# imazen/imageflow

Hardware: NVIDIA B200
Metric: input Mpixels/s, c2_4k_to_512_robidoux (higher is better)
Workload: dtype f32

## Files before the change

imageflow_b200/csrc/ifb_engine.cu:

```cuda
#include <cuda_runtime.h>

#include <algorithm>
#include <atomic>
#include <chrono>
#include <condition_variable>
#include <thread>
#include <cmath>
#include <cstdarg>
#include <cstdio>
#include <cstring>
#include <map>
#include <memory>
#include <mutex>
#include <set>
#include <stdexcept>
#include <string>
#include <tuple>
#include <unordered_map>
#include <vector>

#include "../../include/ifb200.h"
#include "ifb_kernels.cuh"
#include "ifb_weights.h"
#include "ifb_whitespace.h"
// ... 85 lines not shown
    size_t add(const void* src, size_t bytes) {
        const size_t off = (host.size() + 255) / 256 * 256;
        host.resize(off + bytes);
        if (bytes && src) memcpy(host.data() + off, src, bytes);
        return off;
    }
    template <class T> size_t add(const std::vector<T>& v) { return add(v.data(), v.size() * sizeof(T)); }
    size_t add_zeroed(size_t bytes) { return add(nullptr, bytes); }
    template <class T> T* host_at(size_t off) { return reinterpret_cast<T*>(host.data() + off); }
    void reserve(size_t bytes) { host.reserve(bytes); }
    void commit(ifb200_batch* b, cudaStream_t st);
    void use_on(cudaStream_t st) {
        if (done || st == up_stream) return;
        if (cudaEventQuery(ready) == cudaSuccess) { done = true; return; }
        CUDA_OK(cudaStreamWaitEvent(st, ready, 0));
    }
    template <class T> const T* at(size_t off) const { return reinterpret_cast<const T*>(p + off); }
    ~DevBlob() { if (ready && owns_ready) cudaEventDestroy(ready); }
    DevBlob() = default;
    DevBlob(const DevBlob&) = delete;
    DevBlob& operator=(const DevBlob&) = delete;
};

struct AxisOnDev {
    size_t o_left = 0, o_right = 0, o_off = 0, o_w = 0;
    void add_to(DevBlob& blob, const ifb::AxisWeights& a) { o_left = blob.add(a.left); o_right = blob.add(a.right); o_off = blob.add(a.offset); o_w = blob.add(a.w); }
    AxisDev view(const DevBlob& blob) const { return AxisDev{blob.at<uint32_t>(o_left), blob.at<uint32_t>(o_right), blob.at<uint32_t>(o_off), blob.at<float>(o_w)}; }
};

struct HvTables {
    int max_cols = 0, n_strips = 0;
    uint32_t hw_stride = 0;
    std::vector<HvStripDev> strips;
    DevBlob blob;
    size_t o_strips = 0, o_hw = 0, o_hdone = 0, o_vw = 0, o_vdone = 0;
};

struct Plan {
    uint32_t in_w, in_h, out_w, out_h;
    ifb::AxisWeights wv, wh;
    AxisOnDev dv, dh; std::unique_ptr<DevBlob> axes;
    bool tile_ok = false; TilePlanDev tile{};
    std::vector<float> tile_vw, tile_hw; std::vector<uint32_t> tile_vq; size_t o_tile_vw = 0, o_tile_vq = 0, o_tile_hw = 0;
    bool hv_ok = false; std::string hv_reason;
    int av = 0;
    std::map<int, std::unique_ptr<HvTables>> by_cols;
    std::vector<int> cols_failed;
};

bool monotone(const ifb::AxisWeights& a) {
    for (uint32_t i = 1; i < a.out_size; ++i)
        if (a.left[i] < a.left[i - 1] || a.right[i] < a.right[i - 1]) return false;
    return true;
}

int ring_depth(const ifb::AxisWeights& a) {
    int need = 1;
    for (; need <= 64; ++need) {
        bool ok = true;
        for (uint32_t y = 0; y + need < a.out_size && ok; ++y) ok = a.left[y + need] > a.right[y];
        if (ok) break;
    }
    return need;
}

void build_hv(Plan& p) {
// ... 15 lines not shown
        t.max_ic = std::max<int>(t.max_ic, (int)(p.wh.right[X1 - 1] - p.wh.left[X0] + 1));
    }
    for (int ty = 0; ty < t.tiles_y; ++ty) {
        const uint32_t Y0 = ty * t.toh, Y1 = std::min<uint32_t>(Y0 + t.toh, p.out_h);
        t.max_ir = std::max<int>(t.max_ir, (int)(p.wv.right[Y1 - 1] - p.wv.left[Y0] + 1));
    }
    if (Tile2Smem::make(t.max_ir, t.max_ic, true).total > 96u * 1024u) return;
    const int rows_pad = t.tiles_y * kTile2H;
    p.tile_vw.assign((size_t)rows_pad * 8, 0.0f);
    p.tile_vq.assign((size_t)rows_pad / 4, 0u);
    for (int ty = 0; ty < t.tiles_y; ++ty) {
        const uint32_t Y0 = ty * t.toh, Y1 = std::min<uint32_t>(Y0 + t.toh, p.out_h);
        const uint32_t r0 = p.wv.left[Y0], r1 = p.wv.right[Y1 - 1];
        for (uint32_t yq = Y0; yq < Y1; yq += 4) {
            const uint32_t b0 = std::min(p.wv.left[yq], std::max(r1 - std::min<uint32_t>(r1, kTile2Span - 1), r0));
            bool fit = r1 - r0 + 1 >= (uint32_t)kTile2Span;
            for (uint32_t y = yq; y < std::min(yq + 4, Y1); ++y) fit = fit && p.wv.left[y] >= b0 && p.wv.right[y] < b0 + kTile2Span;
            p.tile_vq[yq / 4] = fit ? b0 + 1 : 0u;
            if (!fit) continue;
            for (uint32_t y = yq; y < std::min(yq + 4, Y1); ++y)
                for (uint32_t j = p.wv.left[y]; j <= p.wv.right[y]; ++j) p.tile_vw[(size_t)y * 8 + (j - b0)] = p.wv.w[p.wv.offset[y] + (j - p.wv.left[y])];
        }
    }
    t.h4 = p.wh.max_taps <= 4 ? 1 : 0;
    p.tile_hw.assign(t.h4 ? (size_t)t.tiles_x * kTile2W * 4 : 4, 0.0f);
    if (t.h4)
        for (uint32_t x = 0; x < p.out_w; ++x)
            for (uint32_t j = p.wh.left[x]; j <= p.wh.right[x]; ++j) p.tile_hw[(size_t)x * 4 + (j - p.wh.left[x])] = p.wh.w[p.wh.offset[x] + (j - p.wh.left[x])];
    p.tile = t; p.tile_ok = true;
}

template <class F> void hv_for_av(int av, F&& f) { if (av == 4) f(std::integral_constant<int, 4>{}); else f(std::integral_constant<int, 6>{}); }

std::unique_ptr<HvTables> hv_tables_host(const Plan& p, int cols_key) {
    auto ht = std::make_unique<HvTables>();
    const int max_cols = cols_key & 0xffff, ng = cols_key >> 16, cg = 32 / (p.av / 2);
    ht->max_cols = max_cols;
    const auto& h = p.wh; const auto& v = p.wv;
    const int av = p.av, avp = av == 4 ? 4 : 8, cap = 16384 / (avp * 4);
    const uint32_t col_cap = (uint32_t)max_cols;
    static const uint32_t k0_align = [] { const char* e = getenv("IFB200_DEBUG_K0_ALIGN"); const int v = e ? atoi(e) : 4; return (uint32_t)(v >= 1 && v <= 16 ? v : 4); }();
    auto k0_of = [&](uint32_t X0) { return h.left[X0] / k0_align * k0_align; };
    auto marks_of = [&](uint32_t X0, uint32_t X1, std::vector<uint32_t>* marks) {
        const uint32_t k0 = k0_of(X0);
        uint32_t parked = 0, X = X0, groups = 0;
        const uint32_t npairs = (h.right[X1 - 1] - k0 + 1 + 15) / 16 * 2;
        for (uint32_t c = 0; c < npairs; ++c) {
            uint32_t m = 0;
            while (X < X1 && h.right[X] <= k0 + c * 8 + 7) { ++m; ++X; }
            if (m > (uint32_t)cg) return false;
            if (parked + m > (uint32_t)cg) { if (marks) marks->push_back(c - 1); ++groups; parked = 0; }
            parked += m;
        }
        if (parked) { if (marks) marks->push_back(npairs - 1); ++groups; }
        return groups <= (uint32_t)ng;
    };
    auto fits = [&](uint32_t X0, uint32_t X1) {
        return X1 - X0 <= col_cap && (h.right[X1 - 1] - k0_of(X0) + 1 + 15) / 16 * 16 + 16 <= (uint32_t)cap && marks_of(X0, X1, nullptr);
    };
    uint32_t ns = 0;
    for (uint32_t X0 = 0; X0 < h.out_size; ++ns) {
        uint32_t X1 = X0 + 1;
        if (!fits(X0, X1)) IFB_THROW(IFB200_ERR_INVALID_STATE, "ring kernel: one output column reads %u source columns (> %d)", h.right[X0] - h.left[X0] + 1, cap - 16);
        while (X1 < h.out_size && fits(X0, X1 + 1)) ++X1;
        X0 = X1;
    }
    std::vector<HvStripDev>& strips = ht->strips;
    for (;; ++ns) {
        strips.clear();
        bool ok = true;
        for (uint32_t s = 0; s < ns && ok; ++s) {
            const uint32_t X0 = (uint32_t)((uint64_t)h.out_size * s / ns), X1 = (uint32_t)((uint64_t)h.out_size * (s + 1) / ns);
            if (X1 <= X0) { ok = false; break; }
            ok = fits(X0, X1);
            HvStripDev sd{};
            sd.X0 = (int)X0; sd.X1 = (int)X1; sd.k0 = (int)k0_of(X0);
            sd.nst = (int)((h.right[X1 - 1] - k0_of(X0) + 1 + 15) / 16);
            sd.Xf = (int)X0; sd.hslot0 = (int)(X0 % (uint32_t)av);
            strips.push_back(sd);
        }
        if (ok) break;
        if (ns > h.out_size) IFB_THROW(IFB200_ERR_INVALID_STATE, "ring kernel: strip partition failed");
    }
    ht->n_strips = (int)ns;
    uint32_t rec = 0;
    for (const auto& sd : strips) rec = std::max<uint32_t>(rec, (uint32_t)sd.nst * 16u + 16u);
    ht->hw_stride = rec;
    const size_t hd_stride = (size_t)rec + 64;
    ht->blob.reserve(ns * (sizeof(HvStripDev) + (size_t)rec * avp * 4 + hd_stride) + ((size_t)p.in_h + 32) * (avp * 4 + 1) + 4096);
    ht->o_strips = ht->blob.add(strips);
    ht->o_hw = ht->blob.add_zeroed((size_t)ns * rec * avp * sizeof(float));
    ht->o_hdone = ht->blob.add_zeroed((size_t)ns * hd_stride);
    ht->o_vw = ht->blob.add_zeroed(((size_t)p.in_h + 32) * avp * sizeof(float));
    ht->o_vdone = ht->blob.add_zeroed((size_t)p.in_h + 32);
    float* const hw = ht->blob.host_at<float>(ht->o_hw);
    uint8_t* const hdone = ht->blob.host_at<uint8_t>(ht->o_hdone);
    float* const vw = ht->blob.host_at<float>(ht->o_vw);
    uint8_t* const vdone = ht->blob.host_at<uint8_t>(ht->o_vdone);
    std::vector<uint32_t> marks;
    for (uint32_t s = 0; s < ns; ++s) {
        const HvStripDev& sd = strips[s];
        const uint32_t k0 = (uint32_t)sd.k0;
        for (uint32_t X = (uint32_t)sd.X0; X < (uint32_t)sd.X1; ++X) {
            const float* w = h.w.data() + h.offset[X];
            const uint32_t slot = X % (uint32_t)av;
            for (uint32_t k = h.left[X]; k <= h.right[X]; ++k) hw[((size_t)s * rec + (k - k0)) * avp + slot] = w[k - h.left[X]];
            uint8_t& d = hdone[(size_t)s * hd_stride + (h.right[X] - k0)];
            if (d == 127) IFB_THROW(IFB200_ERR_INVALID_STATE, "ring kernel: too many columns complete at once");
            ++d;
        }
        marks.clear();
        marks_of((uint32_t)sd.X0, (uint32_t)sd.X1, &marks);
        for (uint32_t c : marks) hdone[(size_t)s * hd_stride + c * 8 + 7] |= 0x80u;
    }
    for (uint32_t y = 0; y < v.out_size; ++y) {
        const float* w = v.w.data() + v.offset[y];
        const uint32_t slot = y % (uint32_t)av;
        for (uint32_t j = v.left[y]; j <= v.right[y]; ++j) vw[(size_t)j * avp + slot] = w[j - v.left[y]];
        uint8_t& d = vdone[v.right[y]];
        if (d == 255) IFB_THROW(IFB200_ERR_INVALID_STATE, "ring kernel: too many rows complete at once");
        ++d;
    }
    return ht;
}

bool hv_host_ready(Plan& p, int max_cols) {
    if (!p.hv_ok) return false;
    if (p.by_cols.count(max_cols)) return true;
    if (std::find(p.cols_failed.begin(), p.cols_failed.end(), max_cols) != p.cols_failed.end()) return false;
    try { p.by_cols.emplace(max_cols, hv_tables_host(p, max_cols)); return true; }
    catch (const Err& e) { p.cols_failed.push_back(max_cols); if (p.hv_reason.empty()) p.hv_reason = e.msg; return false; }
}

HvTables& hv_tables(ifb200_batch* bt, cudaStream_t st, Plan& p, int max_cols) {
    auto it = p.by_cols.find(max_cols);
    if (it == p.by_cols.end()) it = p.by_cols.emplace(max_cols, hv_tables_host(p, max_cols)).first;
    HvTables& ht = *it->second;
    if (!ht.blob.p) ht.blob.commit(bt, st); else ht.blob.use_on(st);
    return ht;
}

std::vector<HvBandDev> hv_bands(const Plan& p, int nb) {
    const auto& v = p.wv;
    std::vector<HvBandDev> bands;
    for (int i = 0; i < nb; ++i) {
        const uint32_t Y0 = (uint32_t)((uint64_t)p.out_h * i / nb), Y1 = (uint32_t)((uint64_t)p.out_h * (i + 1) / nb);
// ... 416 lines not shown
            if (g.kind == 1) {
                bl = &p.by_cols.at(g.cols_key)->blob;
            } else {
                if (!p.axes) make_axes_blob(p);
                bl = p.axes.get();
            }
            if (!bl->p && !bl->host.empty() && seen.insert(bl).second) cold.push_back(bl);
        }
    }
    size_t cold_next = 0;
    auto upload_ahead = [&](cudaStream_t up) {
        const size_t end = std::min(cold.size(), cold_next + 128);
        if (cold_next < end) { b->commit_many(up, std::vector<DevBlob*>(cold.begin() + cold_next, cold.begin() + end)); cold_next = end; }
    };
    struct GroupLayout { size_t jobs = 0, tmaps = 0, bands = 0, counters = 0; int nb = 0, grid = 0; std::vector<HvBandDev> bv; };
    std::vector<GroupLayout> lay(groups.size());
    size_t bytes = 0;
    auto take = [&](size_t nbytes) { const size_t o = (bytes + 127) / 128 * 128; bytes = o + nbytes; return o; };
    for (size_t gi = 0; gi < groups.size(); ++gi) {
        Group& g = groups[gi];
        lay[gi].jobs = take(g.idx.size() * sizeof(JobDev));
        if (g.kind == 1) {
            Plan& p = *g.plan;
            const HvEntry* he = find_hv(p.av, g.ch);
            const HvTables& ht = *p.by_cols.at(g.cols_key);
            const size_t jxs = g.idx.size() * (size_t)ht.n_strips;
            const int warps_all = b->sm_count * he->warps;
            const int nb = hv_pick_bands(p, jxs, warps_all, b->min_items);
            lay[gi].bv = hv_bands(p, nb);
            lay[gi].nb = (int)lay[gi].bv.size();
            const size_t items = jxs * nb;
            lay[gi].grid = (int)std::min<size_t>((size_t)b->sm_count, (items + he->warps - 1) / he->warps);
            lay[gi].tmaps = take(g.idx.size() * sizeof(HvTmap));
            lay[gi].bands = take(lay[gi].bv.size() * sizeof(HvBandDev));
            lay[gi].counters = take((size_t)ht.n_strips * sizeof(uint32_t));
        }
    }
    cudaEvent_t ev;
    uint8_t* hbuf = static_cast<uint8_t*>(b->stage(bytes, &ev));
    for (size_t gi = 0; gi < groups.size(); ++gi) {
        Group& g = groups[gi];
        JobDev* hj = reinterpret_cast<JobDev*>(hbuf + lay[gi].jobs);
        HvTmap* ht = g.kind == 1 ? reinterpret_cast<HvTmap*>(hbuf + lay[gi].tmaps) : nullptr;
        size_t pos = 0;
        for (size_t i : g.idx) {
            hj[pos] = make_job(descs[i], g_t_lin_host, g_t_srgb_host);
            if (ht) { uint32_t xoff = 0; ht[pos] = tmap_for(b, descs[i], &xoff); hj[pos].in_xoff = xoff; }
            ++pos;
        }
        if (g.kind == 1) {
            memcpy(hbuf + lay[gi].bands, lay[gi].bv.data(), lay[gi].bv.size() * sizeof(HvBandDev));
            memset(hbuf + lay[gi].counters, 0, (size_t)g.plan->by_cols.at(g.cols_key)->n_strips * sizeof(uint32_t));
        }
    }
    uint8_t* dbuf = nullptr;
    CUDA_OK(cudaMallocAsync(reinterpret_cast<void**>(&dbuf), bytes, st));
    AsyncFree dbuf_guard{dbuf, st};
    CUDA_OK(cudaMemcpyAsync(dbuf, hbuf, bytes, cudaMemcpyHostToDevice, st));
    CUDA_OK(cudaEventRecord(ev, st));

    const bool fork = groups.size() >= 4;
    cudaStream_t const user_stream = st;
    if (fork) {
        CUDA_OK(cudaEventRecord(b->ev_fork, user_stream));
        for (auto& sd : b->side) CUDA_OK(cudaStreamWaitEvent(sd, b->ev_fork, 0));
    }
    struct Join {
        ifb200_batch* b; cudaStream_t user; bool on;
        ~Join() {
            if (!on) return;
            for (int k = 0; k < ifb200_batch::kSideStreams; ++k)
                if (cudaEventRecord(b->ev_join[k], b->side[k]) == cudaSuccess) cudaStreamWaitEvent(user, b->ev_join[k], 0);
        }
    } join{b, user_stream, fork};
    for (size_t gi = 0; gi < groups.size(); ++gi) {
        Group& g = groups[gi];
        Plan& p = *g.plan;
        {
            const DevBlob* need = g.kind == 1 ? &p.by_cols.at(g.cols_key)->blob : p.axes.get();
            while (need && !need->p && cold_next < cold.size()) upload_ahead(user_stream);
        }
        const JobDev* jobs = reinterpret_cast<const JobDev*>(dbuf + lay[gi].jobs);
        const size_t nj = g.idx.size();
        st = fork ? b->side[gi % ifb200_batch::kSideStreams] : user_stream;
// ... 465 lines not shown
                    }
                }
            } catch (const Err& e) { errs[me] = e; }
        };
        const auto t0 = std::chrono::steady_clock::now();
        std::vector<std::thread> pool;
        try { for (int t = 1; t < threads; ++t) pool.emplace_back(worker, t); } catch (...) {}
        worker(0);
        for (auto& th : pool) th.join();
        const double dt = std::chrono::duration<double>(std::chrono::steady_clock::now() - t0).count();
        for (auto& e : errs) if (e.code) throw e;
        if (seconds) *seconds = dt;
        if (table_bytes) *table_bytes = bytes.load();
        if (table_hash) { uint64_t h = 14695981039346656037ull; *table_hash = fnv(h, hashes.data(), hashes.size() * 8); }
    });
}

int ifb200_hv_plan_tables(const ifb200_resample_desc* d, int strip_cols, int n_pairs, ifb200_hv_plan_info* info, uint8_t* buf, size_t cap,
                          char* err, size_t err_cap) {
    return guarded(err, err_cap, [&] {
        if (!d || !info) IFB_THROW(IFB200_ERR_INVALID_ARGUMENT, "null pointer");
        if (strip_cols < 16 || strip_cols > 128 || strip_cols % 16 || n_pairs < 1) IFB_THROW(IFB200_ERR_INVALID_ARGUMENT, "bad strip width or band count");
        memset(info, 0, sizeof *info);
        auto p = ifb200_batch::build_plan_host(*d, strip_cols);
        if (!p->hv_ok) return;
        const int cols = hv_cols(p->av, d->alpha_meaningful ? 4 : 3, strip_cols);
        if (!p->by_cols.count(cols)) return;
        HvTables& ht = *p->by_cols.at(cols);
        const std::vector<HvBandDev> bands = hv_bands(*p, n_pairs);
        const size_t o_bands = (ht.blob.host.size() + 255) / 256 * 256;
        info->ok = 1; info->av = p->av; info->n_strips = ht.n_strips; info->n_bands = (int32_t)bands.size();
        info->avp = p->av == 4 ? 4 : 8; info->cap_px = (int32_t)ht.hw_stride;
        info->o_strips = ht.o_strips; info->o_hw = ht.o_hw; info->o_hdone = ht.o_hdone; info->o_vw = ht.o_vw; info->o_vdone = ht.o_vdone;
        info->o_bands = o_bands; info->total = o_bands + bands.size() * sizeof(HvBandDev);
        if (!buf) return;
        if (cap < info->total) IFB_THROW(IFB200_ERR_CAPACITY, "buffer of %zu bytes, %llu needed", cap, (unsigned long long)info->total);
        memcpy(buf, ht.blob.host.data(), ht.blob.host.size());
        memcpy(buf + o_bands, bands.data(), bands.size() * sizeof(HvBandDev));
    });
}

int  ifb200_color_filter_matrix(int which, float p, float out[25]) { return out ? ifb::color_filter_matrix(which, p, out) : IFB200_ERR_INVALID_ARGUMENT; }

int ifb200_batch_create(int device, ifb200_batch** out, char* err, size_t cap) {
    return guarded(err, cap, [&] {
        if (!out) IFB_THROW(IFB200_ERR_INVALID_ARGUMENT, "null out pointer");
        *out = nullptr;
        *out = create_batch(device);
    });
}

int ifb200_batch_enqueue(ifb200_batch* b, const ifb200_resample_desc* descs, size_t n, void* stream, char* err, size_t cap) {
    return guarded(err, cap, [&] {
        if (!b || (!descs && n)) IFB_THROW(IFB200_ERR_INVALID_ARGUMENT, "null batch or descriptor array");
        std::lock_guard<std::mutex> lk(b->mu);
        enqueue_locked(b, descs, n, stream == IFB200_STREAM_OWN ? b->own_stream : static_cast<cudaStream_t>(stream));
    });
}

int ifb200_batch_color_matrix(ifb200_batch* b, uint8_t* dev_px, uint32_t w, uint32_t h, uint32_t stride, const float m[25],
                              void* stream, char* err, size_t cap) {
    return guarded(err, cap, [&] {
        if (!b) IFB_THROW(IFB200_ERR_INVALID_ARGUMENT, "null batch");
        std::lock_guard<std::mutex> lk(b->mu);
        color_matrix_locked(b, dev_px, w, h, stride, m, stream == IFB200_STREAM_OWN ? b->own_stream : static_cast<cudaStream_t>(stream));
    });
}

int ifb200_batch_apply_matte(ifb200_batch* b, uint8_t* dev_px, uint32_t w, uint32_t h, uint32_t stride, const uint8_t matte_bgra[4],
                             int alpha_meaningful, void* stream, char* err, size_t cap) {
    return guarded(err, cap, [&] {
// ... 362 lines not shown
```

imageflow_b200/csrc/ifb_hv_kernel.cuh:

```cuda
#pragma once

#ifndef IFB_HV_EMU
#include <cuda.h>
#endif

struct HvStripDev { int X0, X1, Xf, hslot0, k0, nst, pad0, pad1; };
struct HvBandDev  { int Y0, Y1, Yf, vslot0, j0, nrows, pad0, pad1; };
struct HvPlanDev {
    uint32_t in_w, in_h, out_w, out_h;
    int n_strips, n_bands;
    const HvStripDev* strips;
    const HvBandDev* bands;
    const float* hw;
    const uint8_t* hdone;
    const float* vw;
    const uint8_t* vdone;
    uint32_t zero;
    uint32_t hw_stride;
};
struct alignas(64) HvTmap { unsigned char bytes[128]; };

#ifndef IFB_HV_MAXCOLS4
#define IFB_HV_MAXCOLS4 64
#endif
template <int AV, int CH> struct HvCfg {
    static_assert(AV == 4 || AV == 6, "ring depth");
    static constexpr int kAvp = AV == 4 ? 4 : 8;
    static constexpr int kCapPx = 16384 / (kAvp * 4);
    static constexpr int kNP = AV / 2;
    static constexpr int kCG = 32 / kNP;
    static constexpr int kMaxCols = AV == 4 ? IFB_HV_MAXCOLS4 : (CH == 3 ? 50 : 40);
    static constexpr int kNG = kMaxCols / kCG + 1;
    static constexpr int kWarps = CH == 3 ? 16 : 12;
    static constexpr int kThreads = kWarps * 32;
    static constexpr int kStages = 2;
    static constexpr int kBoxBytes = 32 * 64;
    static constexpr int kStageBytes = kBoxBytes;
    static constexpr int kRingBytes = kStages * kStageBytes;
    static constexpr int kXPitch = CH * 32 + 2;
    static constexpr int kXBytes = kCG * kXPitch * 4;
};

template <int AV, int CH>
__host__ __device__ constexpr uint32_t hv_layout(uint32_t sb_low16, int warp, uint32_t* st_off, uint32_t* x_off, uint32_t* mb_off) {
    using C = HvCfg<AV, CH>;
    const uint32_t lut_off = (0x10000u - sb_low16) & 0xffffu;
    const uint32_t ring = (uint32_t)C::kRingBytes, xb = (uint32_t)C::kXBytes, W = (uint32_t)C::kWarps;
    const uint32_t a0 = (512u - (sb_low16 & 511u)) & 511u;
    const uint32_t roomA = lut_off > a0 ? lut_off - a0 : 0u;
    uint32_t ra = 0, xa = 0, best = 0;
    for (uint32_t r = 0; r <= W; ++r) {
        if (r * ring > roomA) break;
        uint32_t x = (roomA - r * ring) / xb;
        if (x > W) x = W;
        const uint32_t used = r * ring + x * xb;
        if (used > best) { best = used; ra = r; xa = x; }
    }
    const uint32_t b0 = lut_off + 65536u;
    const uint32_t b_x = b0 + (W - ra) * ring;
    const uint32_t b_mb = (b_x + (W - xa) * xb + 7u) & ~7u;
    if (warp >= 0) {
        const uint32_t w = (uint32_t)warp;
        if (st_off) *st_off = w < ra ? a0 + w * ring : b0 + (w - ra) * ring;
        if (x_off) *x_off = w < xa ? a0 + ra * ring + w * xb : b_x + (w - xa) * xb;
        if (mb_off) *mb_off = b_mb + w * 8u * (uint32_t)C::kStages;
    }
    return b_mb + W * 8u * (uint32_t)C::kStages + 16u;
}
template <int AV, int CH> __host__ __device__ constexpr uint32_t hv_flag_offset(uint32_t sb_low16) { return hv_layout<AV, CH>(sb_low16, -1, nullptr, nullptr, nullptr) - 16u; }
template <int AV, int CH> constexpr uint32_t hv_total_bytes(uint32_t sb_low16) { return hv_layout<AV, CH>(sb_low16, -1, nullptr, nullptr, nullptr); }

#ifndef IFB_HV_EMU
namespace hv {
__device__ __forceinline__ uint32_t smem_u32(const void* p) { return (uint32_t)__cvta_generic_to_shared(p); }
// ... 188 lines not shown
    const uint32_t lane4 = ((uint32_t)lane * 4u) | ((lut >> 16) << 8);
    const uint32_t swz = (((uint32_t)lane >> 1) & 3u) << 4;
    const uint32_t n_bands = (uint32_t)pl.n_bands;
    const uint32_t n_items = n_jobs * n_bands;
    const uint32_t lutw = lut + 128u * 256u + 128u;
    const bool leader = hv::elect_one();
    const uint32_t vh = (uint32_t)lane / (uint32_t)CG, cl = (uint32_t)lane % (uint32_t)CG;
    const bool vlane = vh < (uint32_t)NP;
    const uint32_t xr = xbuf + cl * kXCol;
    const uint32_t xw0 = xbuf + (uint32_t)lane * 4u;

    for (int sv = 0; sv < pl.n_strips; ++sv) {
        if (warp == 0) {
            const int k = sv + lane;
            const bool work = k < pl.n_strips && hv::ldg_volatile(counters + (blockIdx.x + (uint32_t)k) % (uint32_t)pl.n_strips) < n_items;
            const uint32_t m = hv::ballot(work);
            if (lane == 0) hv::sts_u32(flagw, m ? (uint32_t)__ffs((int)m) : (sv + 32 < pl.n_strips ? 33u : 0u));
        }
        hv::cta_sync();
        const uint32_t skip1 = hv::lds_u32(flagw);
        hv::cta_sync();
        if (skip1 == 0u) break;
        if (skip1 == 33u) { sv += 31; continue; }
        sv += (int)skip1 - 1;
        const int s = (int)((blockIdx.x + (uint32_t)sv) % (uint32_t)pl.n_strips);
        const HvStripDev sd_ = pl.strips[s];
        const int sX0 = (int)uni((uint32_t)sd_.X0);
        const uint32_t sH0 = uni((uint32_t)sd_.hslot0);
        const int sK0 = (int)uni((uint32_t)sd_.k0), nst = (int)uni((uint32_t)sd_.nst);
        {
            const float4* __restrict__ src = reinterpret_cast<const float4*>(pl.hw + (size_t)s * pl.hw_stride * AVP);
            const int n16 = (nst * 16 + 4) * AVP / 4;
            for (int u = t; u < n16; u += C::kThreads) hv::sts_f32x4(lutw + ((uint32_t)(u >> 3) << 8) + ((uint32_t)(u & 7) << 4), hv::ldg(src + u));
        }
        hv::cta_sync();
        const uint8_t* __restrict__ hdone = pl.hdone + (size_t)s * (pl.hw_stride + 64u);
        const uint32_t npairs = (uint32_t)nst * 2u;

        for (;;) {
            uint32_t item = 0;
            if (lane == 0) item = hv::atomic_inc(counters + s);
            item = uni(hv::bcast0(item));
            if (item >= n_items) break;
            const uint32_t job_i = item / n_bands, band_i = item - job_i * n_bands;
            const JobDev& job = jobs[job_i];
            const HvTmap* tm = tmaps + job_i;
            const HvBandDev bd_ = pl.bands[band_i];
            const int bJ0 = (int)uni((uint32_t)bd_.j0), bNr = (int)uni((uint32_t)bd_.nrows);
            const int bY0 = (int)uni((uint32_t)bd_.Y0), bY1 = (int)uni((uint32_t)bd_.Y1);
            const uint32_t flags = uni(job.flags);
            const int nrb = (bNr + 31) >> 5;
            const int x_origin = sK0 + (int)uni(job.in_xoff);

            const int x_end = x_origin + nst * 16;
            int tma_x = x_origin, tma_y = bJ0, tma_left = nrb * nst, is_s = 0;
            auto issue = [&](const uint32_t zero_dep) {
                hv::warp_sync();
                if (leader) {
                    const uint32_t bar = mb + 8u * (uint32_t)is_s;
                    hv::mbar_expect_tx(bar, (uint32_t)C::kStageBytes);
                    hv::tma_load_box(stb + (uint32_t)is_s * C::kStageBytes, tm, tma_x + (int)zero_dep, tma_y, bar);
                }
                --tma_left; is_s ^= 1;
                tma_x += 16;
                if (tma_x == x_end) { tma_x = x_origin; tma_y += 32; }
            };
// ... 28 lines not shown
                uint32_t wcur = lutw;

                if (tma_left > 0) issue(0u);
                hv::mbar_wait(mb + 8u * (uint32_t)cs_s, (par >> cs_s) & 1u);
                par ^= 1u << cs_s;
                uint32_t sbase = stb + (uint32_t)cs_s * C::kStageBytes + (uint32_t)lane * 64u;
                uint4 rawA = hv::lds_u32x4(sbase + swz), rawB;
                uint32_t hd_next = (uint32_t)hv::ldg(hdone + lane);
                uint32_t HM1 = 0, HM2 = 0, HMV = 0;

                float P0[CH], P1[CH];
                float2 W0[NP], W1[NP];
                auto conv = [&](float (&P)[CH], const uint32_t v) {
                    P[0] = hv::lut_gather<0x6504>(v, lane4); P[1] = hv::lut_gather<0x6514>(v, lane4); P[2] = hv::lut_gather<0x6524>(v, lane4);
                    if (CH == 4) {
                        const float af = __fmul_rn(__uint2float_rn(v >> 24), 1.0f / 255.0f);
                        P[0] = __fmul_rn(P[0], af); P[1] = __fmul_rn(P[1], af); P[2] = __fmul_rn(P[2], af); P[CH - 1] = af;
                    }
                };
                auto wload = [&](float2 (&W)[NP], const uint32_t a) {
                    const float4 q4 = hv::lds_w4(a);
                    W[0] = make_float2(q4.x, q4.y); W[1] = make_float2(q4.z, q4.w);
                    if (AV == 6) W[NP - 1] = hv::lds_w2(a + 16u);
                };
                auto mac = [&](const float (&P)[CH], const float2 (&W)[NP]) {
#pragma unroll
                    for (int c = 0; c < CH; ++c) {
                        const float2 v_ = make_float2(P[c], P[c]);
#pragma unroll
                        for (int q = 0; q < NP; ++q) accH[c][q] = hv::ffma2(W[q], v_, accH[c][q]);
                    }
                };
                wload(W0, wcur); conv(P0, rawA.x);

                for (uint32_t pq = 0; pq < npairs; pq += 4u) {
                    HM1 = hv::ballot((hd_next & 0x7fu) >= 1u); HM2 = hv::ballot((hd_next & 0x7fu) >= 2u); HMV = hv::ballot((hd_next & 0x80u) != 0u);
                    hd_next = (uint32_t)hv::ldg(hdone + (pq + 4u) * 8u + (uint32_t)lane);
                    const uint32_t pe = min(pq + 4u, npairs);
#pragma unroll 1
                  for (uint32_t pc = pq; pc < pe; ++pc) {
                    const uint32_t hm = HM1, hm2 = HM2, hmv = HMV;
                    HM1 >>= 8; HM2 >>= 8; HMV >>= 8;
                    const uint32_t wB = wcur + (AV == 4 ? 64u : 256u);
                    const uint32_t wnext = wcur + (AV == 4 ? 256u : 512u);
                    const bool more = pc + 1u < npairs;

#define IFB_HV_SLOT(S_) case S_: if (S_ < AV) { _Pragma("unroll") for (int ch_ = 0; ch_ < CH; ++ch_) { \
        float& a_ = (S_ & 1) ? accH[ch_][(S_ % AV) / 2].y : accH[ch_][(S_ % AV) / 2].x; \
        hv::sts_f32(xw + (uint32_t)ch_ * 128u, a_); a_ = 0.0f; } } break;
#define IFB_HV_FLUSH(I_) if ((hm >> (I_)) & 1u) { \
        uint32_t n_ = 1u; \
        if ((hm2 >> (I_)) & 1u) n_ = uni((uint32_t)hv::ldg(hdone + pc * 8u + (I_)) & 0x7fu); \
        _Pragma("unroll 1") do { \
            switch (hslot) { IFB_HV_SLOT(0) IFB_HV_SLOT(1) IFB_HV_SLOT(2) IFB_HV_SLOT(3) IFB_HV_SLOT(4) IFB_HV_SLOT(5) default: break; } \
            xw += kXCol; ++colbuf; hslot = hslot + 1u == (uint32_t)AV ? 0u : hslot + 1u; \
        } while (--n_); }

                    rawB = hv::lds_u32x4(sbase + (((((pc & 1u) << 1) | 1u) << 4) ^ swz));
                    if ((pc & 1u) && more) {
                        cs_s ^= 1;
                        if (tma_left > 0) issue(hv::zero_after(rawB.x, pl.zero));
                        hv::mbar_wait(mb + 8u * (uint32_t)cs_s, (par >> cs_s) & 1u);
                        par ^= 1u << cs_s;
                        sbase = stb + (uint32_t)cs_s * C::kStageBytes + (uint32_t)lane * 64u;
                    }
#define IFB_HV_RELOAD rawA = hv::lds_u32x4(sbase + (((((pc + 1u) & 1u) << 1) << 4) ^ swz));
#define IFB_HV_ACC(S_, C_) (((S_) & 1) ? accH[C_][((S_) % AV) / 2].y : accH[C_][((S_) % AV) / 2].x)
#define IFB_HV_PF(S_, BIT_, M_) { \
        if (CH == 3) hv::flush3_if<BIT_, kXCol>(xw, IFB_HV_ACC(S_, 0), IFB_HV_ACC(S_, 1), IFB_HV_ACC(S_, 2), M_); \
        else hv::flush4_if<BIT_, kXCol>(xw, IFB_HV_ACC(S_, 0), IFB_HV_ACC(S_, 1), IFB_HV_ACC(S_, 2), IFB_HV_ACC(S_, CH - 1), M_); }
#define IFB_HV_NONE
#define IFB_HV_STEPS_A(F0_, F1_, F2_, F3_) { \
        wload(W1, wcur + kRec); conv(P1, rawA.y); mac(P0, W0); F0_ \
        wload(W0, wcur + 2u * kRec); conv(P0, rawA.z); mac(P1, W1); F1_ \
        wload(W1, wcur + 3u * kRec); conv(P1, rawA.w); mac(P0, W0); F2_ \
        wload(W0, wB); conv(P0, rawB.x); mac(P1, W1); F3_ }
#define IFB_HV_STEPS_B(F0_, F1_, F2_, F3_) { \
        wload(W1, wB + kRec); conv(P1, rawB.y); mac(P0, W0); F0_ \
        wload(W0, wB + 2u * kRec); conv(P0, rawB.z); mac(P1, W1); F1_ \
        wload(W1, wB + 3u * kRec); conv(P1, rawB.w); IFB_HV_RELOAD mac(P0, W0); F2_ \
        wload(W0, wnext); conv(P0, rawA.x); mac(P1, W1); F3_ }
#define IFB_HV_CHUNK(STEPS_, SH_) { \
        const uint32_t m4_ = (hm >> (SH_)) & 15u; \
        if (IFB_HV_NOFAST || ((((hm2 >> (SH_)) & 15u) | (m4_ & (m4_ - 1u))) != 0u)) { \
            STEPS_(IFB_HV_FLUSH((SH_) + 0), IFB_HV_FLUSH((SH_) + 1), IFB_HV_FLUSH((SH_) + 2), IFB_HV_FLUSH((SH_) + 3)) \
        } else if (m4_ == 0u) { \
            STEPS_(IFB_HV_NONE, IFB_HV_NONE, IFB_HV_NONE, IFB_HV_NONE) \
        } else { \
            if (hslot < 2u) { \
                if (hslot == 0u) IFB_HV_FORM(STEPS_, 0) else IFB_HV_FORM(STEPS_, 1) \
            } else if (AV == 4 || hslot < 4u) { \
                if (hslot == 2u) IFB_HV_FORM(STEPS_, 2) else IFB_HV_FORM(STEPS_, 3) \
            } else { \
                if (hslot == 4u) IFB_HV_FORM(STEPS_, 4) else IFB_HV_FORM(STEPS_, 5) \
            } \
            ++colbuf; hslot = hslot + 1u == (uint32_t)AV ? 0u : hslot + 1u; \
        } }
#define IFB_HV_FORM(STEPS_, K_) STEPS_(IFB_HV_PF((K_) % AV, 1u, m4_), IFB_HV_PF((K_) % AV, 2u, m4_), IFB_HV_PF((K_) % AV, 4u, m4_), IFB_HV_PF((K_) % AV, 8u, m4_))
                    IFB_HV_CHUNK(IFB_HV_STEPS_A, 0)
                    IFB_HV_CHUNK(IFB_HV_STEPS_B, 4)
#undef IFB_HV_CHUNK
#undef IFB_HV_FORM
#undef IFB_HV_STEPS_A
#undef IFB_HV_STEPS_B
#undef IFB_HV_NONE
#undef IFB_HV_PF
#undef IFB_HV_ACC
#undef IFB_HV_RELOAD
#undef IFB_HV_FLUSH
#undef IFB_HV_SLOT
                    wcur = wnext;

                    if ((hmv >> 7) & 1u) {
                        hv::warp_sync();
                        const bool col_live = vlane && cl < colbuf;
                        uint8_t* const out_px = out_col + (size_t)gX * 4;
                        float2 acc[CH];
                        switch (grp) {
#define IFB_HV_VGROUP(G_) case G_: if (G_ < NG) { _Pragma("unroll") for (int ch_ = 0; ch_ < CH; ++ch_) acc[ch_] = accV[(G_) % NG][ch_]; } break;
                        IFB_HV_VGROUP(0) IFB_HV_VGROUP(1) IFB_HV_VGROUP(2) IFB_HV_VGROUP(3) IFB_HV_VGROUP(4) IFB_HV_VGROUP(5) IFB_HV_VGROUP(6) IFB_HV_VGROUP(7) IFB_HV_VGROUP(8)
#undef IFB_HV_VGROUP
                        default:
#pragma unroll
                            for (int ch_ = 0; ch_ < CH; ++ch_) acc[ch_] = make_float2(0.0f, 0.0f);
                            break;
                        }
                        {
                            int Yb = Yc;
                            uint32_t nc = 0;
                            uint32_t vs = vslot;
                            auto drain = [&]() {
                                hv::warp_sync();
#pragma unroll 1
                                for (uint32_t k0 = 0; k0 < nc; k0 += (uint32_t)NP) {
                                    const uint32_t k = k0 + (vlane ? vh : 0u);
                                    float f_[4] = {0.0f, 0.0f, 0.0f, 0.0f};
#pragma unroll
                                    for (int ch_ = 0; ch_ < CH; ++ch_) f_[ch_] = hv::lds_f32(xr + (uint32_t)ch_ * 128u + (k & 31u) * 4u);
                                    const int Yl = Yb + (int)k;
                                    const bool mine = k < nc && Yl >= bY0 && Yl < bY1 && col_live;
                                    uint8_t* dst = out_px + (size_t)Yl * out_stride;
                                    if (EPI != 0) {
                                        const uint32_t px_ = hv_finish_pixel<EPI, CH>(f_[0], f_[1], f_[2], CH == 4 ? f_[3] : 0.0f, flags, job, lut, lut_lane, dst);
                                        if (mine) *reinterpret_cast<uint32_t*>(dst) = px_;
                                    } else if (mine) {
                                        *reinterpret_cast<uint32_t*>(dst) = hv_finish_pixel<EPI, CH>(f_[0], f_[1], f_[2], CH == 4 ? f_[3] : 0.0f, flags, job, lut, lut_lane, dst);
// ... 31 lines not shown
                                if (n & 1) { vrow(vwp, xrr); vwp += AVP; xrr += 4u; }
                                if (rest != 0u) {
                                    uint32_t nv = 1u;
                                    if (vm2 != 0u && ((vm2 >> (r - 1)) & 1u)) nv = uni((uint32_t)hv::ldg(pl.vdone + row0 + r - 1));
#pragma unroll 1
                                    for (uint32_t e2 = 0; e2 < nv; ++e2) {
                                        if (nc >= (uint32_t)r) drain();
                                        hv::warp_sync();
                                        const bool holder = (vs >> 1) == vh;
                                        const uint32_t pa = xr + nc * 4u;
                                        if (vs & 1u) {
#pragma unroll
                                            for (int ch_ = 0; ch_ < CH; ++ch_) if (holder) { hv::sts_f32(pa + (uint32_t)ch_ * 128u, acc[ch_].y); acc[ch_].y = 0.0f; }
                                        } else {
#pragma unroll
                                            for (int ch_ = 0; ch_ < CH; ++ch_) if (holder) { hv::sts_f32(pa + (uint32_t)ch_ * 128u, acc[ch_].x); acc[ch_].x = 0.0f; }
                                        }
                                        ++nc; vs = vs + 1u == (uint32_t)AV ? 0u : vs + 1u;
                                    }
                                }
                            }
                            drain();
                        }
                        switch (grp) {
#define IFB_HV_VGROUP(G_) case G_: if (G_ < NG) { _Pragma("unroll") for (int ch_ = 0; ch_ < CH; ++ch_) accV[(G_) % NG][ch_] = acc[ch_]; } break;
                        IFB_HV_VGROUP(0) IFB_HV_VGROUP(1) IFB_HV_VGROUP(2) IFB_HV_VGROUP(3) IFB_HV_VGROUP(4) IFB_HV_VGROUP(5) IFB_HV_VGROUP(6) IFB_HV_VGROUP(7) IFB_HV_VGROUP(8)
#undef IFB_HV_VGROUP
                        default: break;
                        }
                        hv::warp_sync();
                        ++grp; gX += colbuf; colbuf = 0; xw = xw0;
                    }
                  }
                }
                cs_s ^= 1;
                Yc += (int)vtot;
                vslot = (vslot + vtot) % (uint32_t)AV;
            }
        }
    }
}
```

Measured before the change: 586,800.

## Add periodic-run fast path with compile-time column completion pattern in HV kernel

On the host, each strip's column-completion pattern is scanned for long runs that match precomputed periodic forms for the 4-tap case. The run offset and length are stored next to the band table. Inside a matched run, the kernel switches to a fully unrolled path whose parking slots are known at compile time, replacing the per-pair ballot masks and runtime branch dispatch. This is meant to cut control overhead in the inner horizontal loop. The cost is larger code and more complex loop bookkeeping, and it only helps when a strip's pattern matches one of the hard-coded forms.

After: 622,100 (median of 6 runs). 1.06x the previous value.

```diff
diff --git a/imageflow_b200/csrc/ifb_engine.cu b/imageflow_b200/csrc/ifb_engine.cu
--- a/imageflow_b200/csrc/ifb_engine.cu
+++ b/imageflow_b200/csrc/ifb_engine.cu
@@ -141,6 +141,7 @@
     int max_cols = 0, n_strips = 0;
     uint32_t hw_stride = 0;
     std::vector<HvStripDev> strips;
+    std::vector<uint32_t> runs;
     DevBlob blob;
     size_t o_strips = 0, o_hw = 0, o_hdone = 0, o_vw = 0, o_vdone = 0;
 };
@@ -222,6 +223,42 @@
 
 template <class F> void hv_for_av(int av, F&& f) { if (av == 4) f(std::integral_constant<int, 4>{}); else f(std::integral_constant<int, 6>{}); }
 
+void hv_find_run(const uint8_t* hd, uint32_t npairs, uint32_t hslot0, int av, int cg, int ng, uint32_t run[2]) {
+    auto pair_done = [&](uint32_t c) { uint32_t d = 0; for (int i = 0; i < 8; ++i) d += hd[c * 8 + i] & 0x7fu; return d; };
+    auto groups_with = [&](uint32_t a, uint32_t P, uint32_t n) {
+        uint32_t parked = 0, groups = 0;
+        for (uint32_t c = 0; c < npairs; ++c) {
+            if (c == a && parked) return -1;
+            parked += pair_done(c);
+            const bool in = c >= a && c < a + n * P;
+            if ((in && (c + 1 - a) % P == 0) || (!in && (hd[c * 8 + 7] & 0x80u) && parked)) { ++groups; parked = 0; }
+        }
+        return (int)groups;
+    };
+    uint32_t best_pairs = 0;
+    for (int f = 0; f < kHvNumForms; ++f) {
+        const HvForm& fm = kHvForms[f];
+        const uint32_t P = (uint32_t)fm.pairs;
+        int tot = 0;
+        for (int i = 0; i < fm.pairs * 8; ++i) tot += fm.cnt[i] - '0';
+        if (fm.av != av || tot > cg) continue;
+        auto period_at = [&](uint32_t c) {
+            for (uint32_t i = 0; i < P * 8; ++i) if ((hd[c * 8 + i] & 0x7fu) != (uint32_t)(fm.cnt[i] - '0')) return false;
+            return true;
+        };
+        uint32_t done = 0;
+        for (uint32_t a = 0; a + P <= npairs; done += pair_done(a), ++a) {
+            if ((hslot0 + done) % (uint32_t)av != (uint32_t)fm.slot) continue;
+            uint32_t n = 0;
+            while (a + (n + 1) * P <= npairs && period_at(a + n * P)) ++n;
+            if (n * P <= best_pairs) continue;
+            const int g = groups_with(a, P, n);
+            if (g < 0 || g > ng) continue;
+            best_pairs = n * P; run[0] = a | (uint32_t)f << 16; run[1] = n;
+        }
+    }
+}
+
 std::unique_ptr<HvTables> hv_tables_host(const Plan& p, int cols_key) {
     auto ht = std::make_unique<HvTables>();
     const int max_cols = cols_key & 0xffff, ng = cols_key >> 16, cg = 32 / (p.av / 2);
@@ -231,6 +268,8 @@
     const uint32_t col_cap = (uint32_t)max_cols;
     static const uint32_t k0_align = [] { const char* e = getenv("IFB200_DEBUG_K0_ALIGN"); const int v = e ? atoi(e) : 4; return (uint32_t)(v >= 1 && v <= 16 ? v : 4); }();
     auto k0_of = [&](uint32_t X0) { return h.left[X0] / k0_align * k0_align; };
+    const char* const pe_ = getenv("IFB200_DEBUG_HV_PERIODIC");
+    const bool periodic = !(pe_ && atoi(pe_) == 0);
     auto marks_of = [&](uint32_t X0, uint32_t X1, std::vector<uint32_t>* marks) {
         const uint32_t k0 = k0_of(X0);
         uint32_t parked = 0, X = X0, groups = 0;
@@ -273,6 +312,7 @@
         if (ns > h.out_size) IFB_THROW(IFB200_ERR_INVALID_STATE, "ring kernel: strip partition failed");
     }
     ht->n_strips = (int)ns;
+    ht->runs.assign(2 * (size_t)ns, 0u);
     uint32_t rec = 0;
     for (const auto& sd : strips) rec = std::max<uint32_t>(rec, (uint32_t)sd.nst * 16u + 16u);
     ht->hw_stride = rec;
@@ -302,6 +342,7 @@
         marks.clear();
         marks_of((uint32_t)sd.X0, (uint32_t)sd.X1, &marks);
         for (uint32_t c : marks) hdone[(size_t)s * hd_stride + c * 8 + 7] |= 0x80u;
+        if (periodic) hv_find_run(hdone + (size_t)s * hd_stride, (uint32_t)sd.nst * 2u, (uint32_t)sd.hslot0, av, cg, ng, &ht->runs[2 * s]);
     }
     for (uint32_t y = 0; y < v.out_size; ++y) {
         const float* w = v.w.data() + v.offset[y];
@@ -784,7 +825,7 @@
             const size_t items = jxs * nb;
             lay[gi].grid = (int)std::min<size_t>((size_t)b->sm_count, (items + he->warps - 1) / he->warps);
             lay[gi].tmaps = take(g.idx.size() * sizeof(HvTmap));
-            lay[gi].bands = take(lay[gi].bv.size() * sizeof(HvBandDev));
+            lay[gi].bands = take(lay[gi].bv.size() * sizeof(HvBandDev) + ht.runs.size() * sizeof(uint32_t));
             lay[gi].counters = take((size_t)ht.n_strips * sizeof(uint32_t));
         }
     }
@@ -802,6 +843,8 @@
         }
         if (g.kind == 1) {
             memcpy(hbuf + lay[gi].bands, lay[gi].bv.data(), lay[gi].bv.size() * sizeof(HvBandDev));
+            const std::vector<uint32_t>& runs = g.plan->by_cols.at(g.cols_key)->runs;
+            memcpy(hbuf + lay[gi].bands + lay[gi].bv.size() * sizeof(HvBandDev), runs.data(), runs.size() * sizeof(uint32_t));
             memset(hbuf + lay[gi].counters, 0, (size_t)g.plan->by_cols.at(g.cols_key)->n_strips * sizeof(uint32_t));
         }
     }
@@ -1333,11 +1376,12 @@
         info->ok = 1; info->av = p->av; info->n_strips = ht.n_strips; info->n_bands = (int32_t)bands.size();
         info->avp = p->av == 4 ? 4 : 8; info->cap_px = (int32_t)ht.hw_stride;
         info->o_strips = ht.o_strips; info->o_hw = ht.o_hw; info->o_hdone = ht.o_hdone; info->o_vw = ht.o_vw; info->o_vdone = ht.o_vdone;
-        info->o_bands = o_bands; info->total = o_bands + bands.size() * sizeof(HvBandDev);
+        info->o_bands = o_bands; info->total = o_bands + bands.size() * sizeof(HvBandDev) + ht.runs.size() * sizeof(uint32_t);
         if (!buf) return;
         if (cap < info->total) IFB_THROW(IFB200_ERR_CAPACITY, "buffer of %zu bytes, %llu needed", cap, (unsigned long long)info->total);
         memcpy(buf, ht.blob.host.data(), ht.blob.host.size());
         memcpy(buf + o_bands, bands.data(), bands.size() * sizeof(HvBandDev));
+        memcpy(buf + o_bands + bands.size() * sizeof(HvBandDev), ht.runs.data(), ht.runs.size() * sizeof(uint32_t));
     });
 }
 
diff --git a/imageflow_b200/csrc/ifb_hv_kernel.cuh b/imageflow_b200/csrc/ifb_hv_kernel.cuh
--- a/imageflow_b200/csrc/ifb_hv_kernel.cuh
+++ b/imageflow_b200/csrc/ifb_hv_kernel.cuh
@@ -40,6 +40,25 @@
     static constexpr int kXPitch = CH * 32 + 2;
     static constexpr int kXBytes = kCG * kXPitch * 4;
 };
+
+struct HvForm { int av, pairs, slot; char cnt[129]; };
+constexpr HvForm kHvForms[] = {
+    {4, 15, 0, "00000010" "00000100" "00000100" "00001000" "00001000" "00010000" "00010000" "00100000"
+               "00100000" "01000000" "01000000" "10000000" "10000001" "00000001" "00000010"},
+    {4, 15, 0, "00100000" "01000000" "01000000" "10000000" "10000001" "00000001" "00000010" "00000010"
+               "00000100" "00000100" "00001000" "00001000" "00010000" "00010000" "00100000"},
+    {4, 8, 0, "01000100" "01000100" "01000100" "01000100" "01000100" "01000100" "01000100" "01000100"},
+};
+constexpr int kHvNumForms = (int)(sizeof(kHvForms) / sizeof(kHvForms[0]));
+__host__ __device__ constexpr int hv_form_done(int f, int n) {
+    int d = 0;
+    for (int i = 0; i < n; ++i) d += kHvForms[f].cnt[i] - '0';
+    return d;
+}
+template <int V> struct HvInt { static constexpr int value = V; };
+template <int B, int E, class F> __host__ __device__ __forceinline__ void hv_unroll(F&& f) {
+    if constexpr (B < E) { f(HvInt<B>{}); hv_unroll<B + 1, E>(f); }
+}
 
 template <int AV, int CH>
 __host__ __device__ constexpr uint32_t hv_layout(uint32_t sb_low16, int warp, uint32_t* st_off, uint32_t* x_off, uint32_t* mb_off) {
@@ -294,6 +313,19 @@
             const float4* __restrict__ src = reinterpret_cast<const float4*>(pl.hw + (size_t)s * pl.hw_stride * AVP);
             const int n16 = (nst * 16 + 4) * AVP / 4;
             for (int u = t; u < n16; u += C::kThreads) hv::sts_f32x4(lutw + ((uint32_t)(u >> 3) << 8) + ((uint32_t)(u & 7) << 4), hv::ldg(src + u));
+            if (t == 0) {
+                const uint32_t* run = reinterpret_cast<const uint32_t*>(pl.bands + pl.n_bands) + 2 * s;
+                const uint32_t rp0 = hv::ldg(run), form = rp0 >> 16, npairs = (uint32_t)nst * 2u;
+                uint32_t nrun = 0;
+                if constexpr (AV == 4)
+                    hv_unroll<0, kHvNumForms>([&](auto fc) {
+                        constexpr int F = decltype(fc)::value;
+                        if (kHvForms[F].av == AV && form == (uint32_t)F) nrun = hv::ldg(run + 1) * (uint32_t)kHvForms[F].pairs;
+                    });
+                hv::sts_u32(flagw + 4u, form);
+                hv::sts_u32(flagw + 8u, nrun ? rp0 & 0xffffu : npairs);
+                hv::sts_u32(flagw + 12u, nrun);
+            }
         }
         hv::cta_sync();
         const uint8_t* __restrict__ hdone = pl.hdone + (size_t)s * (pl.hw_stride + 64u);
@@ -388,14 +420,70 @@
                     }
                 };
                 wload(W0, wcur); conv(P0, rawA.x);
-
-                for (uint32_t pq = 0; pq < npairs; pq += 4u) {
+                auto advance = [&]() {
+                    cs_s ^= 1;
+                    if (tma_left > 0) issue(hv::zero_after(rawB.x, pl.zero));
+                    hv::mbar_wait(mb + 8u * (uint32_t)cs_s, (par >> cs_s) & 1u);
+                    par ^= 1u << cs_s;
+                    sbase = stb + (uint32_t)cs_s * C::kStageBytes + (uint32_t)lane * 64u;
+                };
+                auto period = [&](auto fc, uint32_t& pc) {
+                    constexpr int F = decltype(fc)::value, NPP = kHvForms[F].pairs, TOT = hv_form_done(F, NPP * 8);
+                    static_assert(AV == 4 && kHvForms[F].av == AV && TOT % AV == 0 && TOT <= CG, "a period ends a V group and leaves the ring slot as it was");
+                    hv_unroll<0, NPP>([&](auto jc) {
+                        constexpr int J = decltype(jc)::value;
+                        const uint32_t pj = pc + (uint32_t)J;
+                        const uint32_t w = wcur + (uint32_t)J * 256u;
+                        auto park = [&](auto ic) {
+                            constexpr int I = J * 8 + decltype(ic)::value;
+                            hv_unroll<hv_form_done(F, I), hv_form_done(F, I + 1)>([&](auto kc) {
+                                constexpr int K = decltype(kc)::value, SL = (kHvForms[F].slot + K) % AV;
+#pragma unroll
+                                for (int ch_ = 0; ch_ < CH; ++ch_) {
+                                    float& a_ = (SL & 1) ? accH[ch_][SL / 2].y : accH[ch_][SL / 2].x;
+                                    hv::sts_f32(xw0 + (uint32_t)K * kXCol + (uint32_t)ch_ * 128u, a_); a_ = 0.0f;
+                                }
+                            });
+                        };
+                        rawB = hv::lds_u32x4(sbase + (((((pj & 1u) << 1) | 1u) << 4) ^ swz));
+                        if ((pj & 1u) && pj + 1u < npairs) advance();
+                        wload(W1, w + kRec);      conv(P1, rawA.y); mac(P0, W0); park(HvInt<0>{});
+                        wload(W0, w + 2u * kRec); conv(P0, rawA.z); mac(P1, W1); park(HvInt<1>{});
+                        wload(W1, w + 3u * kRec); conv(P1, rawA.w); mac(P0, W0); park(HvInt<2>{});
+                        wload(W0, w + 4u * kRec); conv(P0, rawB.x); mac(P1, W1); park(HvInt<3>{});
+                        wload(W1, w + 5u * kRec); conv(P1, rawB.y); mac(P0, W0); park(HvInt<4>{});
+                        wload(W0, w + 6u * kRec); conv(P0, rawB.z); mac(P1, W1); park(HvInt<5>{});
+                        wload(W1, w + 7u * kRec); conv(P1, rawB.w);
+                        rawA = hv::lds_u32x4(sbase + (((((pj + 1u) & 1u) << 1) << 4) ^ swz));
+                        mac(P0, W0); park(HvInt<6>{});
+                        wload(W0, w + 256u);      conv(P0, rawA.x); mac(P1, W1); park(HvInt<7>{});
+                    });
+                    wcur += (uint32_t)NPP * 256u;
+                    colbuf = (uint32_t)TOT;
+                    pc += (uint32_t)NPP;
+                };
+
+                uint32_t rnext = hv::lds_u32(flagw + 8u);
+                for (uint32_t pq = 0; pq < npairs;) {
                     HM1 = hv::ballot((hd_next & 0x7fu) >= 1u); HM2 = hv::ballot((hd_next & 0x7fu) >= 2u); HMV = hv::ballot((hd_next & 0x80u) != 0u);
-                    hd_next = (uint32_t)hv::ldg(hdone + (pq + 4u) * 8u + (uint32_t)lane);
-                    const uint32_t pe = min(pq + 4u, npairs);
+                    const bool prd = pq == rnext;
+                    uint32_t nx = pq + 4u;
+                    if (prd) { nx = rnext + hv::lds_u32(flagw + 12u); rnext = npairs; }
+                    hd_next = (uint32_t)hv::ldg(hdone + nx * 8u + (uint32_t)lane);
+                    const uint32_t pe = min(nx, rnext);
 #pragma unroll 1
-                  for (uint32_t pc = pq; pc < pe; ++pc) {
-                    const uint32_t hm = HM1, hm2 = HM2, hmv = HMV;
+                  for (uint32_t pc = pq; pc < pe;) {
+                    uint32_t hmv;
+                    if (prd) {
+                        const uint32_t form = hv::lds_u32(flagw + 4u);
+                        hv_unroll<0, AV == 4 ? kHvNumForms : 0>([&](auto fc) {
+                            if constexpr (kHvForms[decltype(fc)::value].av == AV)
+                                if (form == (uint32_t)decltype(fc)::value) period(fc, pc);
+                        });
+                        hmv = 0x80u;
+                    } else {
+                    const uint32_t hm = HM1, hm2 = HM2;
+                    hmv = HMV;
                     HM1 >>= 8; HM2 >>= 8; HMV >>= 8;
                     const uint32_t wB = wcur + (AV == 4 ? 64u : 256u);
                     const uint32_t wnext = wcur + (AV == 4 ? 256u : 512u);
@@ -413,13 +501,7 @@
         } while (--n_); }
 
                     rawB = hv::lds_u32x4(sbase + (((((pc & 1u) << 1) | 1u) << 4) ^ swz));
-                    if ((pc & 1u) && more) {
-                        cs_s ^= 1;
-                        if (tma_left > 0) issue(hv::zero_after(rawB.x, pl.zero));
-                        hv::mbar_wait(mb + 8u * (uint32_t)cs_s, (par >> cs_s) & 1u);
-                        par ^= 1u << cs_s;
-                        sbase = stb + (uint32_t)cs_s * C::kStageBytes + (uint32_t)lane * 64u;
-                    }
+                    if ((pc & 1u) && more) advance();
 #define IFB_HV_RELOAD rawA = hv::lds_u32x4(sbase + (((((pc + 1u) & 1u) << 1) << 4) ^ swz));
 #define IFB_HV_ACC(S_, C_) (((S_) & 1) ? accH[C_][((S_) % AV) / 2].y : accH[C_][((S_) % AV) / 2].x)
 #define IFB_HV_PF(S_, BIT_, M_) { \
@@ -466,8 +548,10 @@
 #undef IFB_HV_FLUSH
 #undef IFB_HV_SLOT
                     wcur = wnext;
-
-                    if ((hmv >> 7) & 1u) {
+                    ++pc;
+                    }
+
+                    if (((hmv >> 7) & 1u) && colbuf != 0u) {
                         hv::warp_sync();
                         const bool col_live = vlane && cl < colbuf;
                         uint8_t* const out_px = out_col + (size_t)gX * 4;
@@ -565,6 +649,7 @@
                         ++grp; gX += colbuf; colbuf = 0; xw = xw0;
                     }
                   }
+                  pq = pe;
                 }
                 cs_s ^= 1;
                 Yc += (int)vtot;
```
